# Lut99/RayTracer-3

Hardware: NVIDIA B200
Metric: Mrays/s (higher is better)
Workload: dtype f32

## Files before the change

raytracer-3_b200/csrc/rt3_core.cu:

```cuda
#include <algorithm>
#include <cmath>
#include <cstdarg>
#include <cstdio>
#include <cstdlib>
#include <cstring>
#include <atomic>
#include <chrono>
#include <limits>
#include <mutex>
#include <string>
#include <type_traits>
#include <vector>

#include <cub/device/device_radix_sort.cuh>

#include "rt3_kernels.cuh"
#include "rt3_denoise.cuh"
#include "rt3_scene.cuh"
#include "rt3_upload.cuh"

namespace {

thread_local std::string g_error;

// ... 53 lines not shown
    int sm_count = 0;
    cudaStream_t stream = nullptr;
    cudaEvent_t ev_begin = nullptr, ev_end = nullptr, ev_copy = nullptr, ev_k0 = nullptr, ev_k1 = nullptr;
    cudaStream_t last_stream = nullptr;
    bool stats_pending = false;
    bool stats_beam_accel = false;
    bool stats_beam = false;
    bool copy_timed = false;

    bool has_scene = false;
    rt3_scene_view view{};
    uint64_t scene_id = 0;
    DeviceBuffer<float4> pair_xy, filt3, face_rec, spheres, prim_color, materials;
    DeviceBuffer<float2> pair_w;
    DeviceBuffer<uint32_t> prim_material, prim_entity;

    DeviceBuffer<float4> prim_lo, prim_hi, bvh_nodes;
    float centroid_min[3] = { 0, 0, 0 }, centroid_max[3] = { 0, 0, 0 };
    bool bvh_ready = false;
    rt3_bvh_view bvh{};
    double bvh_build_ms = 0.0;

    DeviceBuffer<uint32_t> frame, aov_prim, aov_entity;
    DeviceBuffer<float> aov_t;
    DeviceBuffer<unsigned long long> aov_sums;
    DeviceBuffer<float> aov_albedo, aov_normal;
    DeviceBuffer<unsigned long long> accum, counters;
    rt3_kparams accum_kp{};
    bool accum_valid = false;
    uint32_t accum_first = 0;
// ... 104 lines not shown

template <bool RESIDENT, bool SPHERES_ONLY, bool ACCEL>
int launch_path_aovs(rt3_ctx* ctx, const rt3_camera& cam, const rt3_kparams& kp, size_t smem, uint32_t* prim, uint32_t* ent, float* t,
                     cudaStream_t stream) {
    int rc = configure(path_aov_kernel<RESIDENT, SPHERES_ONLY, ACCEL>, smem, nullptr);
    if (rc != RT3_OK) { return rc; }
    const unsigned long long per_cta = (unsigned long long) RT3_CTA_THREADS * RT3_REF_RAYS;
    const unsigned long long grid = (kp.n_items + per_cta - 1) / per_cta;
    if (grid > 0x7FFFFFFFull) { return fail(RT3_ERR_INVALID, "too many AOV samples in one call (%llu)", kp.n_items); }
    path_aov_kernel<RESIDENT, SPHERES_ONLY, ACCEL><<<(unsigned) grid, RT3_CTA_THREADS, smem, stream>>>(ctx->view, ctx->bvh, cam, kp, ctx->aov_sums.ptr, prim, ent, t,
                                                                                                     ctx->counters.ptr);
    RT3_CUDA(cudaGetLastError());
    return RT3_OK;
}

int build_bvh(rt3_ctx* ctx, cudaStream_t stream) {
    if (ctx->bvh_ready) { return RT3_OK; }
    const uint32_t count[2] = { ctx->view.n_faces, ctx->view.n_spheres }, first[2] = { 0u, ctx->view.n_faces };
    const float margin[2] = { 1.9073486328125e-06f, sqrtf(RT3_FILTER_SLACK) * 1.0001f };
    ctx->bvh.n_prims = ctx->view.n_prims;
    ctx->bvh.nodes = nullptr;
    ctx->bvh_build_ms = 0.0;
    uint32_t node_offset[2] = { 0u, count[0] > 1 ? count[0] - 1 : 0u };
    const size_t n_nodes = (size_t) node_offset[1] + (count[1] > 1 ? count[1] - 1 : 0u);
    for (int w = 0; w < 2; w++) {
        ctx->bvh.tree[w].n_prims = count[w];
        ctx->bvh.tree[w].root = count[w] == 1 ? ~(int32_t) first[w] : (int32_t) node_offset[w];
        ctx->bvh.tree[w].ray_margin = margin[w];
    }
    const uint32_t nmax = count[0] > count[1] ? count[0] : count[1];
// ... 1 lines not shown
    DeviceBuffer<unsigned long long> keys_in, keys_out;
    DeviceBuffer<uint32_t> vals_in, vals_out, arrived;
    DeviceBuffer<int> child, node_parent, leaf_parent;
    DeviceBuffer<float4> box_lo, box_hi;
    DeviceBuffer<unsigned char> temp;
    int rc;
    if ((rc = keys_in.reserve(nmax)) != RT3_OK || (rc = keys_out.reserve(nmax)) != RT3_OK || (rc = vals_in.reserve(nmax)) != RT3_OK ||
        (rc = vals_out.reserve(nmax)) != RT3_OK || (rc = arrived.reserve(nmax)) != RT3_OK || (rc = child.reserve(2 * (size_t) nmax)) != RT3_OK ||
        (rc = node_parent.reserve(nmax)) != RT3_OK || (rc = leaf_parent.reserve(nmax)) != RT3_OK || (rc = box_lo.reserve(nmax)) != RT3_OK ||
        (rc = box_hi.reserve(nmax)) != RT3_OK || (rc = ctx->bvh_nodes.reserve(4 * (n_nodes ? n_nodes : 1))) != RT3_OK) {
        return rc;
    }
    size_t temp_bytes = 0;
    RT3_CUDA(cub::DeviceRadixSort::SortPairs(nullptr, temp_bytes, keys_in.ptr, keys_out.ptr, vals_in.ptr, vals_out.ptr, (int) nmax, 0, 63, stream));
    if ((rc = temp.reserve(temp_bytes ? temp_bytes : 1)) != RT3_OK) { return rc; }
    float3 cmin = make_float3(ctx->centroid_min[0], ctx->centroid_min[1], ctx->centroid_min[2]), cscale;
    {
        const float ex[3] = { ctx->centroid_max[0] - ctx->centroid_min[0], ctx->centroid_max[1] - ctx->centroid_min[1],
                              ctx->centroid_max[2] - ctx->centroid_min[2] };
        cscale = make_float3(ex[0] > 0 ? 1.0f / ex[0] : 0.0f, ex[1] > 0 ? 1.0f / ex[1] : 0.0f, ex[2] > 0 ? 1.0f / ex[2] : 0.0f);
    }
    EventPair ev;
    if ((rc = ev.create()) != RT3_OK) { return rc; }
    RT3_CUDA(cudaEventRecord(ev.begin, stream));
    for (int w = 0; w < 2; w++) {
        const uint32_t n = count[w];
        if (n < 2) { continue; }
        const unsigned grid = (n + 255u) / 256u;
        bvh_morton_kernel<<<grid, 256, 0, stream>>>(n, first[w], ctx->prim_lo.ptr, ctx->prim_hi.ptr, cmin, cscale, keys_in.ptr, vals_in.ptr);
        RT3_CUDA(cudaGetLastError());
        size_t tb = temp_bytes;
        RT3_CUDA(cub::DeviceRadixSort::SortPairs(temp.ptr, tb, keys_in.ptr, keys_out.ptr, vals_in.ptr, vals_out.ptr, (int) n, 0, 63, stream));
        RT3_CUDA(cudaMemsetAsync(arrived.ptr, 0, (size_t) n * sizeof(uint32_t), stream));
        bvh_tree_kernel<<<grid, 256, 0, stream>>>((int) n, keys_out.ptr, child.ptr, node_parent.ptr, leaf_parent.ptr);
        RT3_CUDA(cudaGetLastError());
        bvh_refit_kernel<<<grid, 256, 0, stream>>>((int) n, vals_out.ptr, ctx->prim_lo.ptr, ctx->prim_hi.ptr, child.ptr, node_parent.ptr, leaf_parent.ptr,
// ... 3 lines not shown
    RT3_CUDA(cudaEventRecord(ev.end, stream));
    RT3_CUDA(cudaStreamSynchronize(stream));
    float ms = 0.f;
    RT3_CUDA(cudaEventElapsedTime(&ms, ev.begin, ev.end));
    ctx->bvh_build_ms = ms;
    ctx->bvh.nodes = ctx->bvh_nodes.ptr;
    ctx->bvh_ready = true;
    return RT3_OK;
}

int claim_constant_bank(rt3_ctx* ctx, cudaStream_t stream, std::unique_lock<std::mutex>& lock) {
    if (ctx->device < 0 || ctx->device >= RT3_MAX_DEVICES) { return fail(RT3_ERR_INVALID, "device %d out of range", ctx->device); }
    lock = std::unique_lock<std::mutex>(g_const_mutex[ctx->device]);
    if (g_const_owner[ctx->device] == ctx->scene_id) { return RT3_OK; }
    RT3_CUDA(cudaDeviceSynchronize());
    const size_t pairs = ctx->view.n_prims_padded / 2;
    if (pairs) {
        RT3_CUDA(cudaMemcpyToSymbolAsync(c_pair_xy, ctx->pair_xy.ptr, pairs * sizeof(float4), 0, cudaMemcpyDeviceToDevice, stream));
        RT3_CUDA(cudaMemcpyToSymbolAsync(c_pair_w, ctx->pair_w.ptr, pairs * sizeof(float2), 0, cudaMemcpyDeviceToDevice, stream));
    }
    RT3_CUDA(cudaStreamSynchronize(stream));
    g_const_owner[ctx->device] = ctx->scene_id;
    return RT3_OK;
}

struct trace_plan { bool accel, resident, spheres_only; size_t smem; };

int plan_trace(rt3_ctx* ctx, uint32_t flags, bool path_slots, cudaStream_t stream, trace_plan* plan) {
    plan->accel = (flags & RT3_FLAG_BVH) != 0;
    plan->spheres_only = ctx->view.n_faces == 0;
    if (plan->accel) {
        plan->resident = false;
        plan->smem = rt3_accel_smem_bytes(path_slots);
        return build_bvh(ctx, stream);
// ... 449 lines not shown
template <class T> int stage(DeviceBuffer<unsigned char>& buf, const T* host, size_t bytes, const T** device_view, cudaStream_t stream) {
    if (!host || bytes == 0) { *device_view = nullptr; return RT3_OK; }
    int rc = buf.reserve(bytes);
    if (rc != RT3_OK) { return rc; }
    RT3_CUDA(cudaMemcpyAsync(buf.ptr, host, bytes, cudaMemcpyHostToDevice, stream));
    *device_view = reinterpret_cast<const T*>(buf.ptr);
    return RT3_OK;
}

__global__ void build_init_kernel(rt3_build_info* info) {
    info->error_key = ~0ull; info->n_valid = 0ull; info->ray_slack = 0.f; info->r2_median = 1.0; info->r2_min = 1.0;
    for (int k = 0; k < 4; k++) { info->error_detail[k] = 0u; }
    for (int k = 0; k < 3; k++) { info->cmin_bits[k] = 0x7fffffff; info->cmax_bits[k] = (int) 0x80000000; }
}

int build_scene_on_device(rt3_ctx* ctx, const rt3_scene& d) {
    cudaStream_t stream = ctx->stream;
    ctx->has_scene = false;
    ctx->accum_valid = false;
    ctx->bvh_ready = false;
    const uint32_t nf = d.n_faces, ns = d.n_spheres, np = nf + ns;
    const uint32_t np_pad = (np + RT3_PAD_PRIMS - 1) / RT3_PAD_PRIMS * RT3_PAD_PRIMS;
    int rc;
    auto at_least_one = [](size_t n) { return n ? n : (size_t) 1; };
    if ((rc = ctx->face_rec.reserve(at_least_one(4 * (size_t) nf))) != RT3_OK ||
        (rc = ctx->spheres.reserve(at_least_one(ns))) != RT3_OK || (rc = ctx->prim_color.reserve(at_least_one(np))) != RT3_OK ||
        (rc = ctx->prim_material.reserve(at_least_one(np))) != RT3_OK || (rc = ctx->prim_entity.reserve(at_least_one(np))) != RT3_OK ||
        (rc = ctx->prim_lo.reserve(at_least_one(np))) != RT3_OK || (rc = ctx->prim_hi.reserve(at_least_one(np))) != RT3_OK ||
        (rc = ctx->filt3.reserve(at_least_one(np_pad))) != RT3_OK || (rc = ctx->pair_xy.reserve(at_least_one(np_pad / 2))) != RT3_OK ||
        (rc = ctx->pair_w.reserve(at_least_one(np_pad / 2))) != RT3_OK || (rc = ctx->materials.reserve(at_least_one((size_t) d.n_materials * 2))) != RT3_OK) {
// ... 67 lines not shown
    }
    for (int k = 0; k < 3; k++) {
        float lo = ordered_to_float(h.cmin_bits[k]), hi = ordered_to_float(h.cmax_bits[k]);
        if (!(lo <= hi)) { lo = hi = 0.0f; }
        ctx->centroid_min[k] = lo; ctx->centroid_max[k] = hi;
    }
    rt3_scene_view& v = ctx->view;
    for (int k = 0; k < 3; k++) { v.e1[k] = h.basis[0][k]; v.e2[k] = h.basis[1][k]; v.e3[k] = h.basis[2][k]; }
    v.ray_slack = h.ray_slack;
    ctx->scene_id = g_next_scene_id.fetch_add(1);
    v.n_faces = nf; v.n_spheres = ns; v.n_prims = np; v.n_prims_padded = np_pad;
    v.pair_xy = ctx->pair_xy.ptr; v.pair_w = ctx->pair_w.ptr; v.filt3 = ctx->filt3.ptr;
    v.face_rec = ctx->face_rec.ptr;
    v.spheres = ctx->spheres.ptr; v.prim_color = ctx->prim_color.ptr;
    v.prim_material = ctx->prim_material.ptr; v.prim_entity = ctx->prim_entity.ptr; v.materials = ctx->materials.ptr;
    ctx->has_scene = true;
    return RT3_OK;
}

}

extern "C" {

const char* rt3_last_error(void) { return g_error.c_str(); }

int rt3_create(rt3_ctx** out, int device) {
    if (!out) { return fail(RT3_ERR_INVALID, "out is NULL"); }
    *out = nullptr;
    int n_dev = 0;
    cudaError_t e = cudaGetDeviceCount(&n_dev);
// ... 432 lines not shown
```

raytracer-3_b200/csrc/rt3_device.cuh:

```cuda
#pragma once

#include <cuda_runtime.h>
#include <stdint.h>

#include "rt3cuda.h"
#include "rt3_rng.h"

#ifdef RT3_DEBUG_ASSERTS
#include <assert.h>
#define RT3_ASSERT(cond) assert(cond)
#else
#define RT3_ASSERT(cond) ((void) 0)
#endif

#define RT3_NO_HIT 0xFFFFFFFFu
#define RT3_TMIN 0.001f
#define RT3_ACC_SCALE 16777216.0f

#ifndef RT3_UNROLL_PAIRS
#define RT3_UNROLL_PAIRS 16
#endif
#define RT3_PRAGMA_STR(x) _Pragma(#x)
#define RT3_PRAGMA_UNROLL(n) RT3_PRAGMA_STR(unroll n)
#ifndef RT3_RAYS
#define RT3_RAYS 2
#endif
#ifndef RT3_REF_RAYS
#define RT3_REF_RAYS 2
#endif
#define RT3_WORD_PRIMS 32
#define RT3_PAD_PRIMS 8
#ifndef RT3_CHUNK_WORDS
#define RT3_CHUNK_WORDS 16
#endif
#ifndef RT3_CONST_PRIMS
#define RT3_CONST_PRIMS 768
#endif
#define RT3_TILE_PRIMS 1024
#define RT3_CTA_THREADS 128
#ifndef RT3_CTAS_PER_SM
#define RT3_CTAS_PER_SM 5
#endif
#define RT3_ITEM_CHUNK 256u
#define RT3_ITEM_CHUNK_MIN 32u

#define RT3_FILTER_SLACK 3.814697265625e-06f

struct rt3_vec3 { float x, y, z; };

__device__ __forceinline__ rt3_vec3 v3(float x, float y, float z) { rt3_vec3 r; r.x = x; r.y = y; r.z = z; return r; }
__device__ __forceinline__ rt3_vec3 operator+(rt3_vec3 a, rt3_vec3 b) { return v3(a.x + b.x, a.y + b.y, a.z + b.z); }
__device__ __forceinline__ rt3_vec3 operator-(rt3_vec3 a, rt3_vec3 b) { return v3(a.x - b.x, a.y - b.y, a.z - b.z); }
// ... 12 lines not shown
__device__ __forceinline__ uint32_t unorm8(float c) {
    float m = (c < 0.0f) ? 0.0f : c;
    m = (1.0f < m) ? 1.0f : m;
    if (m != m) { m = 0.0f; }
    return (uint32_t) roundf(m * 255.0f);
}
__device__ __forceinline__ uint32_t pack_rgb(rt3_vec3 c) {
    return (unorm8(c.x) << 24) | (unorm8(c.y) << 16) | (unorm8(c.z) << 8) | 0xFFu;
}

struct rt3_scene_view {
    uint32_t n_faces;
    uint32_t n_spheres;
    uint32_t n_prims;
    uint32_t n_prims_padded;
    const float4* pair_xy;
    const float2* pair_w;
    const float4* filt3;
    const float4* face_rec;
    const float4* spheres;
    const float4* prim_color;
    const uint32_t* prim_material;
    const uint32_t* prim_entity;
    float e1[3], e2[3], e3[3];
    float ray_slack;
    const float4* materials;
};

struct rt3_hit { float t; uint32_t prim; };

// ... 82 lines not shown

template <bool ORDERED>
__device__ __forceinline__ void exact_sphere_path_coherent(uint32_t prim, float4 sp, rt3_vec3 o, rt3_vec3 d, rt3_hit& best) {
    rt3_vec3 oc = o - v3(sp.x, sp.y, sp.z);
    float h = __fmaf_rn(oc.x, d.x, __fmaf_rn(oc.y, d.y, oc.z * d.z));
    float c = __fmaf_rn(oc.x, oc.x, __fmaf_rn(oc.y, oc.y, __fmaf_rn(oc.z, oc.z, -(sp.w * sp.w))));
    float disc = __fmaf_rn(h, h, -c);
    if (disc >= 0.0f) {
        float sq = sqrtf(disc);
        const float t1 = -h - sq, t2 = -h + sq;
        const float t = t1 >= RT3_TMIN ? t1 : t2;
        if (t >= RT3_TMIN && closer<ORDERED>(t, prim, best)) { best.prim = prim; best.t = t; }
    }
}

__constant__ float4 c_pair_xy[RT3_CONST_PRIMS / 2];
__constant__ float2 c_pair_w[RT3_CONST_PRIMS / 2];

#define RT3_MASK_BYTES_FOR(rays) ((rays) * RT3_CHUNK_WORDS * RT3_CTA_THREADS * 4)
#define RT3_MASK_BYTES RT3_MASK_BYTES_FOR(RT3_RAYS)

template <int R>
__device__ __forceinline__ void slab_pair(const float4 A, const float2 B, const float2 (&u1)[R], const float2 (&u2)[R],
                                          const float2 (&nou2)[R], uint32_t (&m)[R]) {
#pragma unroll
    for (int r = 0; r < R; r++) {
        const float2 a = __ffma2_rn(make_float2(A.x, A.y), u1[r], __ffma2_rn(make_float2(A.z, A.w), u2[r], nou2[r]));
        const float2 d = __ffma2_rn(a, a, B);
        m[r] = __funnelshift_l(__float_as_uint(d.x), m[r], 1);
        m[r] = __funnelshift_l(__float_as_uint(d.y), m[r], 1);
    }
}

template <bool CONST_BANK, int R>
__device__ __forceinline__ void sweep_chunk(const float4* __restrict__ xy, const float2* __restrict__ w, uint32_t first_pair, uint32_t n_pairs,
                                            const rt3_ray_filter (&f)[R], uint32_t* __restrict__ masks, uint32_t (&nz)[R]) {
    constexpr uint32_t WORD_PAIRS = RT3_WORD_PRIMS / 2, PAD_PAIRS = RT3_PAD_PRIMS / 2;
    float2 nou2[R], u1[R], u2[R];
#pragma unroll
    for (int r = 0; r < R; r++) {
        nou2[r] = make_float2(f[r].nou, f[r].nou); u1[r] = make_float2(f[r].u1, f[r].u1); u2[r] = make_float2(f[r].u2, f[r].u2);
        nz[r] = 0u;
    }
    uint32_t waddr = smem_u32(masks) + threadIdx.x * 4u;
    auto emit = [&](const uint32_t (&m)[R]) {
#pragma unroll
        for (int r = 0; r < R; r++) {
            asm volatile("st.shared.u32 [%0], %1;" ::"r"(waddr + (uint32_t) (r * RT3_CHUNK_WORDS * RT3_CTA_THREADS * 4)), "r"(m[r]) : "memory");
            asm("{ .reg .u32 t; add.cc.u32 t, %1, 0xFFFFFFFF; addc.u32 %0, %0, %0; }" : "+r"(nz[r]) : "r"(m[r]));
        }
        waddr += RT3_CTA_THREADS * 4u;
    };
    const uint32_t n_full = n_pairs / WORD_PAIRS;
    uint32_t base = first_pair;
    for (uint32_t wd = 0; wd < n_full; wd++, base += WORD_PAIRS) {
        uint32_t m[R];
#pragma unroll
        for (int r = 0; r < R; r++) { m[r] = 0u; }
RT3_PRAGMA_UNROLL(RT3_UNROLL_PAIRS)
        for (int j = 0; j < (int) WORD_PAIRS; j++) {
            slab_pair<R>(CONST_BANK ? c_pair_xy[base + j] : xy[base + j], CONST_BANK ? c_pair_w[base + j] : w[base + j], u1, u2, nou2, m);
        }
        emit(m);
    }
    const uint32_t left = n_pairs - n_full * WORD_PAIRS;
    if (left) {
        uint32_t m[R];
#pragma unroll
        for (int r = 0; r < R; r++) { m[r] = 0u; }
        for (uint32_t g = 0; g < left; g += PAD_PAIRS) {
#pragma unroll
            for (int j = 0; j < (int) PAD_PAIRS; j++) {
                slab_pair<R>(CONST_BANK ? c_pair_xy[base + g + j] : xy[base + g + j], CONST_BANK ? c_pair_w[base + g + j] : w[base + g + j], u1, u2, nou2, m);
            }
        }
#pragma unroll
        for (int r = 0; r < R; r++) { m[r] <<= 32u - 2u * left; }
        emit(m);
    }
}

template <bool PATH_MODE, bool SPHERES_ONLY>
__device__ __forceinline__ void drain_chunk(const rt3_scene_view& S, uint32_t first_prim, uint32_t n_words, const rt3_ray_filter& f, rt3_vec3 o,
                                            rt3_vec3 d, const uint32_t* __restrict__ masks, uint32_t nz, rt3_hit& best) {
    uint32_t m = 0u, word_prim = 0u;
    const uint32_t maddr = smem_u32(masks);
    for (;;) {
        if (m == 0u) {
            if (nz == 0u) { break; }
            const uint32_t b = 31u - (uint32_t) __clz((int) nz);
            nz ^= 1u << b;
            const uint32_t wd = n_words - 1u - b;
            RT3_ASSERT(b < n_words && n_words <= RT3_CHUNK_WORDS);
            asm volatile("ld.shared.u32 %0, [%1];" : "=r"(m) : "r"(maddr + wd * (RT3_CTA_THREADS * 4u)));
            word_prim = first_prim + wd * RT3_WORD_PRIMS;
        }
        const uint32_t k = (uint32_t) __clz((int) m);
        m ^= 0x80000000u >> k;
        const uint32_t prim = word_prim + k;
        RT3_ASSERT(prim < S.n_prims);
        if (SPHERES_ONLY || prim >= S.n_faces) {
            const float4 sp = __ldg(&S.spheres[SPHERES_ONLY ? prim : prim - S.n_faces]);
            if (PATH_MODE) { exact_sphere_path<true>(prim, sp, o, d, best); }
            else { exact_sphere_v4<true>(prim, sp, o, d, best); }
        } else {
            if (line_test(__ldg(&S.filt3[prim]), f)) { exact_face<true>(S, prim, o, d, PATH_MODE ? RT3_TMIN : 0.0f, best); }
        }
    }
}

template <bool PATH_MODE, bool CONST_BANK, bool SPHERES_ONLY, int R>
__device__ __forceinline__ void sweep_range(const rt3_scene_view& S, const float4* __restrict__ xy, const float2* __restrict__ w, uint32_t first_pair,
                                            uint32_t first_prim, uint32_t n_prims, const rt3_ray_filter (&f)[R],
                                            const rt3_vec3 (&o)[R], const rt3_vec3 (&d)[R], const bool (&live)[R],
                                            uint32_t* __restrict__ masks, rt3_hit (&best)[R]) {
    constexpr uint32_t CHUNK_PAIRS = RT3_CHUNK_WORDS * RT3_WORD_PRIMS / 2;
    const uint32_t n_pairs = n_prims / 2;
    for (uint32_t p0 = 0, w0 = 0; p0 < n_pairs; p0 += CHUNK_PAIRS, w0 += RT3_CHUNK_WORDS) {
        uint32_t nz[R];
        const uint32_t np = n_pairs - p0 < CHUNK_PAIRS ? n_pairs - p0 : CHUNK_PAIRS;
        sweep_chunk<CONST_BANK, R>(xy, w, first_pair + p0, np, f, masks, nz);
#pragma unroll
        for (int r = 0; r < R; r++) {
            if (!live[r]) { nz[r] = 0u; }
            drain_chunk<PATH_MODE, SPHERES_ONLY>(S, first_prim + w0 * RT3_WORD_PRIMS, (np + RT3_WORD_PRIMS / 2 - 1) / (RT3_WORD_PRIMS / 2), f[r], o[r], d[r],
                                                 masks + r * RT3_CHUNK_WORDS * RT3_CTA_THREADS + threadIdx.x, nz[r], best[r]);
        }
    }
}



__device__ __forceinline__ void mbar_init(uint64_t* bar, uint32_t count) {
    asm volatile("mbarrier.init.shared::cta.b64 [%0], %1;" ::"r"(smem_u32(bar)), "r"(count) : "memory");
}
__device__ __forceinline__ void mbar_expect_tx(uint64_t* bar, uint32_t bytes) {
    asm volatile("mbarrier.arrive.expect_tx.shared::cta.b64 _, [%0], %1;" ::"r"(smem_u32(bar)), "r"(bytes) : "memory");
}
__device__ __forceinline__ void mbar_wait(uint64_t* bar, uint32_t parity) {
    asm volatile(
// ... 15 lines not shown
```

raytracer-3_b200/csrc/rt3_kernels.cuh:

```cuda
#pragma once

#include "rt3_device.cuh"
#include "rt3_bvh.cuh"

struct rt3_kparams {
    uint32_t width, height;
    uint32_t spp, max_depth, seed, flags;
    uint32_t first_sample;
    uint32_t resolve_spp;
    uint32_t tile_rows, part_index, part_count;
    uint32_t owned_rows;
    unsigned long long n_pixels;
    unsigned long long n_items;
    uint32_t resident;
};

__device__ __forceinline__ uint32_t owned_row_to_global(const rt3_kparams& P, uint32_t local_row) {
    uint32_t lt = local_row / P.tile_rows, within = local_row - lt * P.tile_rows;
    return (lt * P.part_count + P.part_index) * P.tile_rows + within;
}

struct rt3_smem_view {
    uint64_t* bars;
    float4* tile_xy;
// ... 57 lines not shown
    bulk_copy_g2s(sm.tile_w + (size_t) stage * RT3_TILE_PAIRS, S.pair_w + first_pair, n * 8u, &sm.bars[stage]);
}

template <bool PATH_MODE, bool RESIDENT, bool SPHERES_ONLY, int R>
__device__ __forceinline__ void sweep_scene(const rt3_scene_view& S, const rt3_smem_view& sm, uint32_t& phase,
                                            const rt3_vec3 (&o)[R], const rt3_vec3 (&d)[R], const rt3_vec3 (&dn)[R],
                                            const bool (&live)[R], rt3_hit (&best)[R]) {
    rt3_ray_filter f[R];
#pragma unroll
    for (int r = 0; r < R; r++) {
        f[r] = make_ray_filter(S, o[r], dn[r]);
        best[r].t = __int_as_float(0x7f800000);
        best[r].prim = RT3_NO_HIT;
    }
    if (RESIDENT) {
        sweep_range<PATH_MODE, true, SPHERES_ONLY, R>(S, nullptr, nullptr, 0u, 0u, S.n_prims_padded, f, o, d, live, sm.masks, best);
        return;
    }
    const uint32_t n_tiles = (S.n_prims_padded + RT3_TILE_PRIMS - 1) / RT3_TILE_PRIMS;
    if (threadIdx.x == 0 && n_tiles > 0) { fetch_tile(S, sm, 0u, 0u); }
    for (uint32_t t = 0; t < n_tiles; t++) {
        const uint32_t stage = t & 1u;
        if (threadIdx.x == 0 && t + 1 < n_tiles) { fetch_tile(S, sm, t + 1, stage ^ 1u); }
        mbar_wait(&sm.bars[stage], (phase >> stage) & 1u);
        phase ^= 1u << stage;
        const uint32_t first = t * RT3_TILE_PRIMS;
        const uint32_t n = S.n_prims_padded - first < RT3_TILE_PRIMS ? S.n_prims_padded - first : RT3_TILE_PRIMS;
        sweep_range<PATH_MODE, false, SPHERES_ONLY, R>(S, sm.tile_xy + (size_t) stage * RT3_TILE_PAIRS, sm.tile_w + (size_t) stage * RT3_TILE_PAIRS, 0u, first, n,
                                      f, o, d, live, sm.masks, best);
        __syncthreads();
    }
// ... 21 lines not shown

#ifdef RT3_SURVIVOR_STATS
__device__ unsigned long long g_survivor_stats[4];
__device__ __forceinline__ void count_survivors(const uint32_t* __restrict__ masks, uint32_t n_words, uint32_t nz, bool live) {
    uint32_t mine = 0;
    for (uint32_t wd = 0; wd < n_words; wd++) { if ((nz >> (n_words - 1u - wd)) & 1u) { mine += (uint32_t) __popc(masks[wd * RT3_CTA_THREADS]); } }
    const uint32_t total = __reduce_add_sync(0xffffffffu, mine), most = __reduce_max_sync(0xffffffffu, mine);
    const uint32_t lanes = (uint32_t) __popc(__ballot_sync(0xffffffffu, live));
    if ((threadIdx.x & 31) == 0) {
        atomicAdd(&g_survivor_stats[0], (unsigned long long) total); atomicAdd(&g_survivor_stats[1], (unsigned long long) most);
        atomicAdd(&g_survivor_stats[2], 1ull); atomicAdd(&g_survivor_stats[3], (unsigned long long) lanes);
    }
}
#endif

template <bool SPHERES_ONLY>
__device__ __forceinline__ void drain_slots(const rt3_scene_view& S, const rt3_smem_view& sm, uint32_t first_prim, uint32_t n_pairs,
                                            const rt3_ray_filter (&f)[RT3_RAYS], const uint32_t (&nz)[RT3_RAYS]) {
    const uint32_t n_words = (n_pairs + RT3_WORD_PRIMS / 2 - 1) / (RT3_WORD_PRIMS / 2);
    static_assert(RT3_RAYS * RT3_CHUNK_WORDS <= 64, "survivor summaries are packed into 64 bits");
    unsigned long long packed = 0ull;
#pragma unroll
    for (int r = 0; r < RT3_RAYS; r++) { packed |= (unsigned long long) nz[r] << (r * RT3_CHUNK_WORDS); }
#pragma unroll 1
    for (int r = 0; r < RT3_RAYS; r++) {
        const uint32_t mine = (uint32_t) (packed >> (r * RT3_CHUNK_WORDS)) & ((1u << RT3_CHUNK_WORDS) - 1u);
        rt3_hit best;
        best.t = slot_float(sm, r, RT3_F_BEST_T); best.prim = slot_word(sm, r, RT3_F_BEST_PRIM);
        rt3_ray_filter fr = f[0];
        const rt3_vec3 o = slot_vec(sm, r, RT3_F_OX), d = slot_vec(sm, r, RT3_F_DX);
        if (!SPHERES_ONLY) { fr = make_ray_filter(S, o, d); }
#ifdef RT3_SURVIVOR_STATS
        count_survivors(sm.masks + r * RT3_CHUNK_WORDS * RT3_CTA_THREADS + threadIdx.x, n_words, mine, slot_word(sm, r, RT3_F_BOUNCE) != RT3_NO_HIT);
#endif
        drain_chunk<true, SPHERES_ONLY>(S, first_prim, n_words, fr, o, d, sm.masks + r * RT3_CHUNK_WORDS * RT3_CTA_THREADS + threadIdx.x, mine, best);
        slot_word(sm, r, RT3_F_BEST_T) = __float_as_uint(best.t); slot_word(sm, r, RT3_F_BEST_PRIM) = best.prim;
    }
}

template <bool RESIDENT, bool SPHERES_ONLY>
__device__ __forceinline__ void sweep_slots(const rt3_scene_view& S, const rt3_smem_view& sm, uint32_t& phase) {
    constexpr uint32_t CHUNK_PAIRS = RT3_CHUNK_WORDS * RT3_WORD_PRIMS / 2;
    rt3_ray_filter f[RT3_RAYS];
    slot_filters(S, sm, f);
#pragma unroll
    for (int r = 0; r < RT3_RAYS; r++) { slot_word(sm, r, RT3_F_BEST_T) = 0x7f800000u; slot_word(sm, r, RT3_F_BEST_PRIM) = RT3_NO_HIT; }
    if (RESIDENT) {
        const uint32_t n_pairs = S.n_prims_padded / 2;
        for (uint32_t p0 = 0; p0 < n_pairs; p0 += CHUNK_PAIRS) {
            uint32_t nz[RT3_RAYS];
            const uint32_t np = n_pairs - p0 < CHUNK_PAIRS ? n_pairs - p0 : CHUNK_PAIRS;
            sweep_chunk<true, RT3_RAYS>(nullptr, nullptr, p0, np, f, sm.masks, nz);
            drain_slots<SPHERES_ONLY>(S, sm, 2u * p0, np, f, nz);
        }
        return;
    }
    const uint32_t n_tiles = (S.n_prims_padded + RT3_TILE_PRIMS - 1) / RT3_TILE_PRIMS;
    if (threadIdx.x == 0 && n_tiles > 0) { fetch_tile(S, sm, 0u, 0u); }
    for (uint32_t t = 0; t < n_tiles; t++) {
        const uint32_t stage = t & 1u;
        if (threadIdx.x == 0 && t + 1 < n_tiles) { fetch_tile(S, sm, t + 1, stage ^ 1u); }
        mbar_wait(&sm.bars[stage], (phase >> stage) & 1u);
        phase ^= 1u << stage;
        const uint32_t first = t * RT3_TILE_PRIMS;
        const uint32_t n_pairs = (S.n_prims_padded - first < RT3_TILE_PRIMS ? S.n_prims_padded - first : RT3_TILE_PRIMS) / 2;
        const float4* xy = sm.tile_xy + (size_t) stage * RT3_TILE_PAIRS;
        const float2* w = sm.tile_w + (size_t) stage * RT3_TILE_PAIRS;
        for (uint32_t p0 = 0; p0 < n_pairs; p0 += CHUNK_PAIRS) {
            uint32_t nz[RT3_RAYS];
            const uint32_t np = n_pairs - p0 < CHUNK_PAIRS ? n_pairs - p0 : CHUNK_PAIRS;
            sweep_chunk<false, RT3_RAYS>(xy, w, p0, np, f, sm.masks, nz);
            drain_slots<SPHERES_ONLY>(S, sm, first + 2u * p0, np, f, nz);
        }
        __syncthreads();
    }
}

__device__ __forceinline__ uint32_t& slot_word_at(const rt3_smem_view& sm, uint32_t r, int field, uint32_t t) {
    return sm.slots[(r * RT3_SLOT_FIELDS + field) * RT3_CTA_THREADS + t];
}
__device__ __forceinline__ rt3_vec3 slot_vec_at(const rt3_smem_view& sm, uint32_t r, int field, uint32_t t) {
    return v3(__uint_as_float(slot_word_at(sm, r, field, t)), __uint_as_float(slot_word_at(sm, r, field + 1, t)), __uint_as_float(slot_word_at(sm, r, field + 2, t)));
}

#ifndef RT3_TAIL_RAYS
#define RT3_TAIL_RAYS 8
#endif
// ... 894 lines not shown
                filled += n_made;
                if (!slot_turn && !__any_sync(0xffffffffu, got)) { break; }
            }
            bool any = false;
#pragma unroll
            for (int r = 0; r < R; r++) { any = any || slot_word(sm, r, RT3_F_BOUNCE) != RT3_NO_HIT; }
            if (!__any_sync(0xffffffffu, any)) {
                if (chunk.dry) { break; }
                continue;
            }
            if constexpr (ACCEL) {
                if (BIN == 2) { traverse_slots_warp_sorted<false>(S, B, sm, bin, visits, tests); }
                else if (BIN == 3) { traverse_slots_warp_sorted<true>(S, B, sm, bin, visits, tests); }
                else { traverse_slots(S, B, sm, visits, tests); }
            } else {
                if (chunk.dry && warp_live_slots(sm) <= RT3_TAIL_RAYS) { sweep_slots_by_primitive(S, sm); }
                else { sweep_slots<RESIDENT, SPHERES_ONLY>(S, sm, phase); }
            }
        }
    } else
    for (;;) {
#pragma unroll 1
        for (int r = 0; r < R; r++) {
            rt3_path s;
            s.bounce = slot_word(sm, r, RT3_F_BOUNCE);
            if (s.bounce != RT3_NO_HIT) {
                s.o = slot_vec(sm, r, RT3_F_OX); s.d = slot_vec(sm, r, RT3_F_DX); s.thr = slot_vec(sm, r, RT3_F_TX);
                s.key = slot_word(sm, r, RT3_F_KEY); s.pix = slot_word(sm, r, RT3_F_PIX);
                rt3_hit best;
                best.t = slot_float(sm, r, RT3_F_BEST_T); best.prim = slot_word(sm, r, RT3_F_BEST_PRIM);
                rays++;
                shade_path(s, best, S, P, accum);
// ... 48 lines not shown
            }
            __syncwarp();
        }
        if (BIN == 1) {
            if (!traverse_slots_binned(S, B, sm, bin, visits, tests)) { break; }
            continue;
        }
        bool any = false;
#pragma unroll
        for (int r = 0; r < R; r++) { any = any || slot_word(sm, r, RT3_F_BOUNCE) != RT3_NO_HIT; }
        if (RESIDENT) { if (!__any_sync(0xffffffffu, any)) { break; } }
        else { if (!__syncthreads_or(any ? 1 : 0)) { break; } }
        if (BIN == 2) { traverse_slots_warp_sorted<false>(S, B, sm, bin, visits, tests); }
        else if (BIN == 3) { traverse_slots_warp_sorted<true>(S, B, sm, bin, visits, tests); }
        else if (ACCEL) { traverse_slots(S, B, sm, visits, tests); }
        else if (RESIDENT && chunk.dry && warp_live_slots(sm) <= RT3_TAIL_RAYS) { sweep_slots_by_primitive(S, sm); }
        else { sweep_slots<RESIDENT, SPHERES_ONLY>(S, sm, phase); }
    }
    for (int off = 16; off > 0; off >>= 1) { rays += __shfl_down_sync(0xffffffffu, rays, off); }
    if ((threadIdx.x & 31) == 0 && rays) { atomicAdd(&counters[1], rays); }
    if (ACCEL) { count_accel(visits, tests, counters); }
    if (BEAM) {
        unsigned long long br = beam_rays, bt = beam_tests;
        for (int off = 16; off > 0; off >>= 1) { br += __shfl_down_sync(0xffffffffu, br, off); bt += __shfl_down_sync(0xffffffffu, bt, off); }
        if ((threadIdx.x & 31) == 0 && br) { atomicAdd(&counters[ACCEL ? 5 : 2], br); atomicAdd(&counters[ACCEL ? 6 : 3], bt); }
    }
}


__device__ __forceinline__ long long to_fixed_signed(float c) {
    float s = c * RT3_ACC_SCALE;
// ... 218 lines not shown
```

raytracer-3_b200/csrc/rt3_upload.cuh:

```cuda
#pragma once

#include "rt3_device.cuh"

struct rt3_build_info {
    unsigned long long error_key;
    uint32_t error_detail[4];
    unsigned long long n_valid;
    float basis[3][3];
    float ray_slack;
    int cmin_bits[3], cmax_bits[3];
    double r2_median, r2_min;
};

#define RT3_BUILD_ERR_VERTEX 0u
#define RT3_BUILD_ERR_MATERIAL 1u
#define RT3_BUILD_ERR_KIND 2u

struct rt3_bound { double cx, cy, cz, R2; };

__device__ __forceinline__ int float_to_ordered(float f) { const int i = __float_as_int(f); return i >= 0 ? i : i ^ 0x7fffffff; }
__host__ __device__ inline float ordered_to_float(int i) {
    const int b = i >= 0 ? i : i ^ 0x7fffffff;
#if defined(__CUDA_ARCH__)
    return __int_as_float(b);
// ... 258 lines not shown
    pair_xy[j] = make_float4(a.x, b.x, a.y, b.y);
    pair_w[j] = make_float2(a.w, b.w);
#pragma unroll
    for (uint32_t k = 0; k < 2u; k++) {
        const uint32_t prim = 2u * j + k;
        if (prim >= n_prims) { continue; }
        const float4 lo = prim_lo[prim], hi = prim_hi[prim];
        if (!(lo.x <= hi.x)) { continue; }
        const float c[3] = { 0.5f * lo.x + 0.5f * hi.x, 0.5f * lo.y + 0.5f * hi.y, 0.5f * lo.z + 0.5f * hi.z };
#pragma unroll
        for (int ax = 0; ax < 3; ax++) {
            if (isfinite(c[ax])) { atomicMin(&info->cmin_bits[ax], float_to_ordered(c[ax])); atomicMax(&info->cmax_bits[ax], float_to_ordered(c[ax])); }
        }
    }
}
```

Before: 11410.

## Reorder constant bank by Morton code and cull 32-prim words via bounding spheres

Builds a constant-memory bank in which large primitives come first and the rest follow in Morton-sorted order. Each 32-primitive word gets a bounding sphere. The resident sweep first computes a per-ray reach mask against these word spheres, then skips slab testing for words no lane in the warp can reach. Drain maps bank slots back to primitive ids through a uint16 table. This is meant to cut slab work for spatially coherent scenes, at the cost of an extra per-ray word pass, an indirection load, and giving up ordered hit tie-breaking.

```diff
diff --git a/raytracer-3_b200/csrc/rt3_core.cu b/raytracer-3_b200/csrc/rt3_core.cu
--- a/raytracer-3_b200/csrc/rt3_core.cu
+++ b/raytracer-3_b200/csrc/rt3_core.cu
@@ -91,6 +91,9 @@
     DeviceBuffer<float4> pair_xy, filt3, face_rec, spheres, prim_color, materials;
     DeviceBuffer<float2> pair_w;
     DeviceBuffer<uint32_t> prim_material, prim_entity;
+    DeviceBuffer<float4> bank_xy, bank_words;
+    DeviceBuffer<float2> bank_w;
+    DeviceBuffer<uint16_t> bank_prim;
 
     DeviceBuffer<float4> prim_lo, prim_hi, bvh_nodes;
     float centroid_min[3] = { 0, 0, 0 }, centroid_max[3] = { 0, 0, 0 };
@@ -225,6 +228,13 @@
     return RT3_OK;
 }
 
+void morton_frame(const rt3_ctx* ctx, float3* cmin, float3* cscale) {
+    *cmin = make_float3(ctx->centroid_min[0], ctx->centroid_min[1], ctx->centroid_min[2]);
+    const float ex[3] = { ctx->centroid_max[0] - ctx->centroid_min[0], ctx->centroid_max[1] - ctx->centroid_min[1],
+                          ctx->centroid_max[2] - ctx->centroid_min[2] };
+    *cscale = make_float3(ex[0] > 0 ? 1.0f / ex[0] : 0.0f, ex[1] > 0 ? 1.0f / ex[1] : 0.0f, ex[2] > 0 ? 1.0f / ex[2] : 0.0f);
+}
+
 int build_bvh(rt3_ctx* ctx, cudaStream_t stream) {
     if (ctx->bvh_ready) { return RT3_OK; }
     const uint32_t count[2] = { ctx->view.n_faces, ctx->view.n_spheres }, first[2] = { 0u, ctx->view.n_faces };
@@ -256,12 +266,8 @@
     size_t temp_bytes = 0;
     RT3_CUDA(cub::DeviceRadixSort::SortPairs(nullptr, temp_bytes, keys_in.ptr, keys_out.ptr, vals_in.ptr, vals_out.ptr, (int) nmax, 0, 63, stream));
     if ((rc = temp.reserve(temp_bytes ? temp_bytes : 1)) != RT3_OK) { return rc; }
-    float3 cmin = make_float3(ctx->centroid_min[0], ctx->centroid_min[1], ctx->centroid_min[2]), cscale;
-    {
-        const float ex[3] = { ctx->centroid_max[0] - ctx->centroid_min[0], ctx->centroid_max[1] - ctx->centroid_min[1],
-                              ctx->centroid_max[2] - ctx->centroid_min[2] };
-        cscale = make_float3(ex[0] > 0 ? 1.0f / ex[0] : 0.0f, ex[1] > 0 ? 1.0f / ex[1] : 0.0f, ex[2] > 0 ? 1.0f / ex[2] : 0.0f);
-    }
+    float3 cmin, cscale;
+    morton_frame(ctx, &cmin, &cscale);
     EventPair ev;
     if ((rc = ev.create()) != RT3_OK) { return rc; }
     RT3_CUDA(cudaEventRecord(ev.begin, stream));
@@ -295,10 +301,11 @@
     lock = std::unique_lock<std::mutex>(g_const_mutex[ctx->device]);
     if (g_const_owner[ctx->device] == ctx->scene_id) { return RT3_OK; }
     RT3_CUDA(cudaDeviceSynchronize());
-    const size_t pairs = ctx->view.n_prims_padded / 2;
+    const size_t pairs = ctx->view.n_bank_recs / 2;
     if (pairs) {
-        RT3_CUDA(cudaMemcpyToSymbolAsync(c_pair_xy, ctx->pair_xy.ptr, pairs * sizeof(float4), 0, cudaMemcpyDeviceToDevice, stream));
-        RT3_CUDA(cudaMemcpyToSymbolAsync(c_pair_w, ctx->pair_w.ptr, pairs * sizeof(float2), 0, cudaMemcpyDeviceToDevice, stream));
+        RT3_CUDA(cudaMemcpyToSymbolAsync(c_pair_xy, ctx->bank_xy.ptr, pairs * sizeof(float4), 0, cudaMemcpyDeviceToDevice, stream));
+        RT3_CUDA(cudaMemcpyToSymbolAsync(c_pair_w, ctx->bank_w.ptr, pairs * sizeof(float2), 0, cudaMemcpyDeviceToDevice, stream));
+        RT3_CUDA(cudaMemcpyToSymbolAsync(c_word_sphere, ctx->bank_words.ptr, ctx->view.n_bank_words * sizeof(float4), 0, cudaMemcpyDeviceToDevice, stream));
     }
     RT3_CUDA(cudaStreamSynchronize(stream));
     g_const_owner[ctx->device] = ctx->scene_id;
@@ -778,6 +785,46 @@
     for (int k = 0; k < 3; k++) { info->cmin_bits[k] = 0x7fffffff; info->cmax_bits[k] = (int) 0x80000000; }
 }
 
+int build_bank(rt3_ctx* ctx, const rt3_bound* bounds, const rt3_build_info* info) {
+    cudaStream_t stream = ctx->stream;
+    const uint32_t n = ctx->view.n_prims;
+    DeviceBuffer<unsigned long long> keys_in, keys_out;
+    DeviceBuffer<uint32_t> vals_in, vals_out, counts;
+    DeviceBuffer<unsigned char> temp;
+    int rc;
+    if ((rc = keys_in.reserve(n)) != RT3_OK || (rc = keys_out.reserve(n)) != RT3_OK || (rc = vals_in.reserve(n)) != RT3_OK ||
+        (rc = vals_out.reserve(n)) != RT3_OK || (rc = counts.reserve(2)) != RT3_OK || (rc = ctx->bank_prim.reserve(RT3_BANK_RECS)) != RT3_OK ||
+        (rc = ctx->bank_xy.reserve(RT3_BANK_RECS / 2)) != RT3_OK || (rc = ctx->bank_w.reserve(RT3_BANK_RECS / 2)) != RT3_OK ||
+        (rc = ctx->bank_words.reserve(RT3_BANK_WORDS)) != RT3_OK) {
+        return rc;
+    }
+    size_t temp_bytes = 0;
+    RT3_CUDA(cub::DeviceRadixSort::SortPairs(nullptr, temp_bytes, keys_in.ptr, keys_out.ptr, vals_in.ptr, vals_out.ptr, (int) n, 0, 64, stream));
+    if ((rc = temp.reserve(temp_bytes ? temp_bytes : 1)) != RT3_OK) { return rc; }
+    float3 cmin, cscale;
+    morton_frame(ctx, &cmin, &cscale);
+    const unsigned grid = (n + 255u) / 256u;
+    RT3_CUDA(cudaMemsetAsync(counts.ptr, 0, 2 * sizeof(uint32_t), stream));
+    bvh_morton_kernel<<<grid, 256, 0, stream>>>(n, 0u, ctx->prim_lo.ptr, ctx->prim_hi.ptr, cmin, cscale, keys_in.ptr, vals_in.ptr);
+    RT3_CUDA(cudaGetLastError());
+    build_bank_keys_kernel<<<grid, 256, 0, stream>>>(n, bounds, info, keys_in.ptr, counts.ptr);
+    RT3_CUDA(cudaGetLastError());
+    RT3_CUDA(cub::DeviceRadixSort::SortPairs(temp.ptr, temp_bytes, keys_in.ptr, keys_out.ptr, vals_in.ptr, vals_out.ptr, (int) n, 0, 64, stream));
+    build_bank_records_kernel<<<(RT3_BANK_RECS / 2 + 127) / 128, 128, 0, stream>>>(n, vals_out.ptr, ctx->filt3.ptr, counts.ptr, ctx->bank_prim.ptr,
+                                                                                    ctx->bank_xy.ptr, ctx->bank_w.ptr);
+    RT3_CUDA(cudaGetLastError());
+    build_bank_words_kernel<<<1, 32, 0, stream>>>(counts.ptr, ctx->bank_prim.ptr, bounds, ctx->filt3.ptr, ctx->bank_words.ptr);
+    RT3_CUDA(cudaGetLastError());
+    uint32_t h[2] = { 0u, 0u };
+    RT3_CUDA(cudaMemcpyAsync(h, counts.ptr, sizeof h, cudaMemcpyDeviceToHost, stream));
+    RT3_CUDA(cudaStreamSynchronize(stream));
+    if (h[1] > RT3_BANK_RECS || h[1] < n) { return fail(RT3_ERR_INVALID, "constant-bank layout of %u records for %u primitives", h[1], n); }
+    ctx->view.n_bank_recs = h[1];
+    ctx->view.n_bank_words = (h[1] + RT3_WORD_PRIMS - 1) / RT3_WORD_PRIMS;
+    ctx->view.bank_prim = ctx->bank_prim.ptr;
+    return RT3_OK;
+}
+
 int build_scene_on_device(rt3_ctx* ctx, const rt3_scene& d) {
     cudaStream_t stream = ctx->stream;
     ctx->has_scene = false;
@@ -875,6 +922,8 @@
     v.face_rec = ctx->face_rec.ptr;
     v.spheres = ctx->spheres.ptr; v.prim_color = ctx->prim_color.ptr;
     v.prim_material = ctx->prim_material.ptr; v.prim_entity = ctx->prim_entity.ptr; v.materials = ctx->materials.ptr;
+    v.n_bank_recs = 0; v.n_bank_words = 0; v.bank_prim = nullptr;
+    if (np && np_pad <= RT3_CONST_PRIMS && (rc = build_bank(ctx, bounds.ptr, info.ptr)) != RT3_OK) { return rc; }
     ctx->has_scene = true;
     return RT3_OK;
 }
diff --git a/raytracer-3_b200/csrc/rt3_device.cuh b/raytracer-3_b200/csrc/rt3_device.cuh
--- a/raytracer-3_b200/csrc/rt3_device.cuh
+++ b/raytracer-3_b200/csrc/rt3_device.cuh
@@ -36,6 +36,9 @@
 #ifndef RT3_CONST_PRIMS
 #define RT3_CONST_PRIMS 768
 #endif
+#define RT3_BANK_RECS (RT3_CONST_PRIMS + RT3_WORD_PRIMS)
+#define RT3_BANK_WORDS (RT3_BANK_RECS / RT3_WORD_PRIMS)
+#define RT3_BANK_PAD 0xFFFFu
 #define RT3_TILE_PRIMS 1024
 #define RT3_CTA_THREADS 128
 #ifndef RT3_CTAS_PER_SM
@@ -78,6 +81,9 @@
     uint32_t n_spheres;
     uint32_t n_prims;
     uint32_t n_prims_padded;
+    uint32_t n_bank_recs;
+    uint32_t n_bank_words;
+    const uint16_t* bank_prim;
     const float4* pair_xy;
     const float2* pair_w;
     const float4* filt3;
@@ -190,8 +196,9 @@
     }
 }
 
-__constant__ float4 c_pair_xy[RT3_CONST_PRIMS / 2];
-__constant__ float2 c_pair_w[RT3_CONST_PRIMS / 2];
+__constant__ float4 c_pair_xy[RT3_BANK_RECS / 2];
+__constant__ float2 c_pair_w[RT3_BANK_RECS / 2];
+__constant__ float4 c_word_sphere[RT3_BANK_WORDS];
 
 #define RT3_MASK_BYTES_FOR(rays) ((rays) * RT3_CHUNK_WORDS * RT3_CTA_THREADS * 4)
 #define RT3_MASK_BYTES RT3_MASK_BYTES_FOR(RT3_RAYS)
@@ -208,9 +215,9 @@
     }
 }
 
-template <bool CONST_BANK, int R>
+template <bool CONST_BANK, int R, bool SKIP = false>
 __device__ __forceinline__ void sweep_chunk(const float4* __restrict__ xy, const float2* __restrict__ w, uint32_t first_pair, uint32_t n_pairs,
-                                            const rt3_ray_filter (&f)[R], uint32_t* __restrict__ masks, uint32_t (&nz)[R]) {
+                                            const rt3_ray_filter (&f)[R], uint32_t* __restrict__ masks, uint32_t (&nz)[R], uint32_t visit = ~0u) {
     constexpr uint32_t WORD_PAIRS = RT3_WORD_PRIMS / 2, PAD_PAIRS = RT3_PAD_PRIMS / 2;
     float2 nou2[R], u1[R], u2[R];
 #pragma unroll
@@ -233,9 +240,11 @@
         uint32_t m[R];
 #pragma unroll
         for (int r = 0; r < R; r++) { m[r] = 0u; }
+        if (!SKIP || __any_sync(0xffffffffu, (int) (visit << wd) < 0)) {
 RT3_PRAGMA_UNROLL(RT3_UNROLL_PAIRS)
-        for (int j = 0; j < (int) WORD_PAIRS; j++) {
-            slab_pair<R>(CONST_BANK ? c_pair_xy[base + j] : xy[base + j], CONST_BANK ? c_pair_w[base + j] : w[base + j], u1, u2, nou2, m);
+            for (int j = 0; j < (int) WORD_PAIRS; j++) {
+                slab_pair<R>(CONST_BANK ? c_pair_xy[base + j] : xy[base + j], CONST_BANK ? c_pair_w[base + j] : w[base + j], u1, u2, nou2, m);
+            }
         }
         emit(m);
     }
@@ -244,7 +253,8 @@
         uint32_t m[R];
 #pragma unroll
         for (int r = 0; r < R; r++) { m[r] = 0u; }
-        for (uint32_t g = 0; g < left; g += PAD_PAIRS) {
+        const bool any_left = !SKIP || __any_sync(0xffffffffu, (int) (visit << n_full) < 0);
+        for (uint32_t g = 0; any_left && g < left; g += PAD_PAIRS) {
 #pragma unroll
             for (int j = 0; j < (int) PAD_PAIRS; j++) {
                 slab_pair<R>(CONST_BANK ? c_pair_xy[base + g + j] : xy[base + g + j], CONST_BANK ? c_pair_w[base + g + j] : w[base + g + j], u1, u2, nou2, m);
@@ -256,9 +266,10 @@
     }
 }
 
-template <bool PATH_MODE, bool SPHERES_ONLY>
+template <bool PATH_MODE, bool SPHERES_ONLY, bool BANK>
 __device__ __forceinline__ void drain_chunk(const rt3_scene_view& S, uint32_t first_prim, uint32_t n_words, const rt3_ray_filter& f, rt3_vec3 o,
                                             rt3_vec3 d, const uint32_t* __restrict__ masks, uint32_t nz, rt3_hit& best) {
+    constexpr bool ORDERED = !BANK;
     uint32_t m = 0u, word_prim = 0u;
     const uint32_t maddr = smem_u32(masks);
     for (;;) {
@@ -273,14 +284,14 @@
         }
         const uint32_t k = (uint32_t) __clz((int) m);
         m ^= 0x80000000u >> k;
-        const uint32_t prim = word_prim + k;
+        const uint32_t prim = BANK ? (uint32_t) __ldg(&S.bank_prim[word_prim + k]) : word_prim + k;
         RT3_ASSERT(prim < S.n_prims);
         if (SPHERES_ONLY || prim >= S.n_faces) {
             const float4 sp = __ldg(&S.spheres[SPHERES_ONLY ? prim : prim - S.n_faces]);
-            if (PATH_MODE) { exact_sphere_path<true>(prim, sp, o, d, best); }
-            else { exact_sphere_v4<true>(prim, sp, o, d, best); }
+            if (PATH_MODE) { exact_sphere_path<ORDERED>(prim, sp, o, d, best); }
+            else { exact_sphere_v4<ORDERED>(prim, sp, o, d, best); }
         } else {
-            if (line_test(__ldg(&S.filt3[prim]), f)) { exact_face<true>(S, prim, o, d, PATH_MODE ? RT3_TMIN : 0.0f, best); }
+            if (line_test(__ldg(&S.filt3[prim]), f)) { exact_face<ORDERED>(S, prim, o, d, PATH_MODE ? RT3_TMIN : 0.0f, best); }
         }
     }
 }
@@ -299,7 +310,7 @@
 #pragma unroll
         for (int r = 0; r < R; r++) {
             if (!live[r]) { nz[r] = 0u; }
-            drain_chunk<PATH_MODE, SPHERES_ONLY>(S, first_prim + w0 * RT3_WORD_PRIMS, (np + RT3_WORD_PRIMS / 2 - 1) / (RT3_WORD_PRIMS / 2), f[r], o[r], d[r],
+            drain_chunk<PATH_MODE, SPHERES_ONLY, CONST_BANK>(S, first_prim + w0 * RT3_WORD_PRIMS, (np + RT3_WORD_PRIMS / 2 - 1) / (RT3_WORD_PRIMS / 2), f[r], o[r], d[r],
                                                  masks + r * RT3_CHUNK_WORDS * RT3_CTA_THREADS + threadIdx.x, nz[r], best[r]);
         }
     }
diff --git a/raytracer-3_b200/csrc/rt3_kernels.cuh b/raytracer-3_b200/csrc/rt3_kernels.cuh
--- a/raytracer-3_b200/csrc/rt3_kernels.cuh
+++ b/raytracer-3_b200/csrc/rt3_kernels.cuh
@@ -95,7 +95,7 @@
         best[r].prim = RT3_NO_HIT;
     }
     if (RESIDENT) {
-        sweep_range<PATH_MODE, true, SPHERES_ONLY, R>(S, nullptr, nullptr, 0u, 0u, S.n_prims_padded, f, o, d, live, sm.masks, best);
+        sweep_range<PATH_MODE, true, SPHERES_ONLY, R>(S, nullptr, nullptr, 0u, 0u, S.n_bank_recs, f, o, d, live, sm.masks, best);
         return;
     }
     const uint32_t n_tiles = (S.n_prims_padded + RT3_TILE_PRIMS - 1) / RT3_TILE_PRIMS;
@@ -147,7 +147,7 @@
 }
 #endif
 
-template <bool SPHERES_ONLY>
+template <bool SPHERES_ONLY, bool BANK>
 __device__ __forceinline__ void drain_slots(const rt3_scene_view& S, const rt3_smem_view& sm, uint32_t first_prim, uint32_t n_pairs,
                                             const rt3_ray_filter (&f)[RT3_RAYS], const uint32_t (&nz)[RT3_RAYS]) {
     const uint32_t n_words = (n_pairs + RT3_WORD_PRIMS / 2 - 1) / (RT3_WORD_PRIMS / 2);
@@ -166,28 +166,71 @@
 #ifdef RT3_SURVIVOR_STATS
         count_survivors(sm.masks + r * RT3_CHUNK_WORDS * RT3_CTA_THREADS + threadIdx.x, n_words, mine, slot_word(sm, r, RT3_F_BOUNCE) != RT3_NO_HIT);
 #endif
-        drain_chunk<true, SPHERES_ONLY>(S, first_prim, n_words, fr, o, d, sm.masks + r * RT3_CHUNK_WORDS * RT3_CTA_THREADS + threadIdx.x, mine, best);
+        drain_chunk<true, SPHERES_ONLY, BANK>(S, first_prim, n_words, fr, o, d, sm.masks + r * RT3_CHUNK_WORDS * RT3_CTA_THREADS + threadIdx.x, mine, best);
         slot_word(sm, r, RT3_F_BEST_T) = __float_as_uint(best.t); slot_word(sm, r, RT3_F_BEST_PRIM) = best.prim;
     }
 }
 
+__device__ __forceinline__ void word_reach(const rt3_scene_view& S, const rt3_smem_view& sm, uint32_t (&reach)[RT3_RAYS]) {
+    float ox[RT3_RAYS], oy[RT3_RAYS], oz[RT3_RAYS], dx[RT3_RAYS], dy[RT3_RAYS], dz[RT3_RAYS], omega[RT3_RAYS];
+#pragma unroll
+    for (int r = 0; r < RT3_RAYS; r++) {
+        ox[r] = slot_float(sm, r, RT3_F_OX); oy[r] = slot_float(sm, r, RT3_F_OY); oz[r] = slot_float(sm, r, RT3_F_OZ);
+        dx[r] = slot_float(sm, r, RT3_F_DX); dy[r] = slot_float(sm, r, RT3_F_DY); dz[r] = slot_float(sm, r, RT3_F_DZ);
+        const float dd = __fmaf_rn(dx[r], dx[r], __fmaf_rn(dy[r], dy[r], dz[r] * dz[r]));
+        omega[r] = __fmaf_rn(S.ray_slack, __fmaf_rn(ox[r], ox[r], __fmaf_rn(oy[r], oy[r], oz[r] * oz[r])), 1.0f);
+        if (!(fabsf(dd - 1.0f) <= 9.5367431640625e-07f)) { omega[r] = __int_as_float(0x7fc00000); }
+        reach[r] = 0u;
+    }
+#pragma unroll 1
+    for (uint32_t k = 0; k < S.n_bank_words; k++) {
+        const float4 w = c_word_sphere[k];
+#pragma unroll
+        for (int r = 0; r < RT3_RAYS; r++) {
+            const float cx = w.x - ox[r], cy = w.y - oy[r], cz = w.z - oz[r];
+            const float tc = __fmaf_rn(cx, dx[r], __fmaf_rn(cy, dy[r], cz * dz[r]));
+            const float L = __fmaf_rn(cx, cx, __fmaf_rn(cy, cy, cz * cz));
+            const float lim = __fmaf_rn(L, 1.52587890625e-05f, w.w * omega[r]);
+            const bool drop = __fmaf_rn(-tc, tc, L) > lim || (tc < 0.0f && L > lim);
+            reach[r] = 2u * reach[r] + (drop ? 0u : 1u);
+        }
+    }
+#pragma unroll
+    for (int r = 0; r < RT3_RAYS; r++) {
+        reach[r] = S.n_bank_words ? reach[r] << (32u - S.n_bank_words) : 0u;
+        if (slot_word(sm, r, RT3_F_BOUNCE) == RT3_NO_HIT) { reach[r] = 0u; }
+    }
+}
+
 template <bool RESIDENT, bool SPHERES_ONLY>
-__device__ __forceinline__ void sweep_slots(const rt3_scene_view& S, const rt3_smem_view& sm, uint32_t& phase) {
+__device__ __forceinline__ void sweep_slots(const rt3_scene_view& S, const rt3_smem_view& sm, uint32_t& phase, bool done = false) {
     constexpr uint32_t CHUNK_PAIRS = RT3_CHUNK_WORDS * RT3_WORD_PRIMS / 2;
     rt3_ray_filter f[RT3_RAYS];
     slot_filters(S, sm, f);
-#pragma unroll
-    for (int r = 0; r < RT3_RAYS; r++) { slot_word(sm, r, RT3_F_BEST_T) = 0x7f800000u; slot_word(sm, r, RT3_F_BEST_PRIM) = RT3_NO_HIT; }
     if (RESIDENT) {
-        const uint32_t n_pairs = S.n_prims_padded / 2;
-        for (uint32_t p0 = 0; p0 < n_pairs; p0 += CHUNK_PAIRS) {
+        uint32_t reach[RT3_RAYS], visit = 0u;
+        word_reach(S, sm, reach);
+#pragma unroll
+        for (int r = 0; r < RT3_RAYS; r++) {
+            if (done) { reach[r] = 0u; }
+            else { slot_word(sm, r, RT3_F_BEST_T) = 0x7f800000u; slot_word(sm, r, RT3_F_BEST_PRIM) = RT3_NO_HIT; }
+            visit |= reach[r];
+        }
+
+        const uint32_t n_pairs = S.n_bank_recs / 2;
+        for (uint32_t p0 = 0, w0 = 0; p0 < n_pairs; p0 += CHUNK_PAIRS, w0 += RT3_CHUNK_WORDS) {
             uint32_t nz[RT3_RAYS];
             const uint32_t np = n_pairs - p0 < CHUNK_PAIRS ? n_pairs - p0 : CHUNK_PAIRS;
-            sweep_chunk<true, RT3_RAYS>(nullptr, nullptr, p0, np, f, sm.masks, nz);
-            drain_slots<SPHERES_ONLY>(S, sm, 2u * p0, np, f, nz);
+            const uint32_t n_words = (np + RT3_WORD_PRIMS / 2 - 1) / (RT3_WORD_PRIMS / 2);
+            sweep_chunk<true, RT3_RAYS, true>(nullptr, nullptr, p0, np, f, sm.masks, nz, visit << w0);
+#pragma unroll
+            for (int r = 0; r < RT3_RAYS; r++) { nz[r] &= (reach[r] << w0) >> (32u - n_words); }
+            drain_slots<SPHERES_ONLY, true>(S, sm, 2u * p0, np, f, nz);
         }
         return;
     }
+#pragma unroll
+    for (int r = 0; r < RT3_RAYS; r++) { slot_word(sm, r, RT3_F_BEST_T) = 0x7f800000u; slot_word(sm, r, RT3_F_BEST_PRIM) = RT3_NO_HIT; }
     const uint32_t n_tiles = (S.n_prims_padded + RT3_TILE_PRIMS - 1) / RT3_TILE_PRIMS;
     if (threadIdx.x == 0 && n_tiles > 0) { fetch_tile(S, sm, 0u, 0u); }
     for (uint32_t t = 0; t < n_tiles; t++) {
@@ -203,7 +246,7 @@
             uint32_t nz[RT3_RAYS];
             const uint32_t np = n_pairs - p0 < CHUNK_PAIRS ? n_pairs - p0 : CHUNK_PAIRS;
             sweep_chunk<false, RT3_RAYS>(xy, w, p0, np, f, sm.masks, nz);
-            drain_slots<SPHERES_ONLY>(S, sm, first + 2u * p0, np, f, nz);
+            drain_slots<SPHERES_ONLY, false>(S, sm, first + 2u * p0, np, f, nz);
         }
         __syncthreads();
     }
@@ -1128,8 +1171,9 @@
                 else if (BIN == 3) { traverse_slots_warp_sorted<true>(S, B, sm, bin, visits, tests); }
                 else { traverse_slots(S, B, sm, visits, tests); }
             } else {
-                if (chunk.dry && warp_live_slots(sm) <= RT3_TAIL_RAYS) { sweep_slots_by_primitive(S, sm); }
-                else { sweep_slots<RESIDENT, SPHERES_ONLY>(S, sm, phase); }
+                const bool tail = chunk.dry && warp_live_slots(sm) <= RT3_TAIL_RAYS;
+                if (tail) { sweep_slots_by_primitive(S, sm); }
+                sweep_slots<RESIDENT, SPHERES_ONLY>(S, sm, phase, tail);
             }
         }
     } else
@@ -1208,7 +1252,11 @@
         if (BIN == 2) { traverse_slots_warp_sorted<false>(S, B, sm, bin, visits, tests); }
         else if (BIN == 3) { traverse_slots_warp_sorted<true>(S, B, sm, bin, visits, tests); }
         else if (ACCEL) { traverse_slots(S, B, sm, visits, tests); }
-        else if (RESIDENT && chunk.dry && warp_live_slots(sm) <= RT3_TAIL_RAYS) { sweep_slots_by_primitive(S, sm); }
+        else if (RESIDENT) {
+            const bool tail = chunk.dry && warp_live_slots(sm) <= RT3_TAIL_RAYS;
+            if (tail) { sweep_slots_by_primitive(S, sm); }
+            sweep_slots<RESIDENT, SPHERES_ONLY>(S, sm, phase, tail);
+        }
         else { sweep_slots<RESIDENT, SPHERES_ONLY>(S, sm, phase); }
     }
     for (int off = 16; off > 0; off >>= 1) { rays += __shfl_down_sync(0xffffffffu, rays, off); }
diff --git a/raytracer-3_b200/csrc/rt3_upload.cuh b/raytracer-3_b200/csrc/rt3_upload.cuh
--- a/raytracer-3_b200/csrc/rt3_upload.cuh
+++ b/raytracer-3_b200/csrc/rt3_upload.cuh
@@ -296,3 +296,67 @@
         }
     }
 }
+
+#define RT3_BANK_LARGE_R2 16.0
+
+__global__ void build_bank_keys_kernel(uint32_t n, const rt3_bound* __restrict__ bounds, const rt3_build_info* __restrict__ info,
+                                       unsigned long long* __restrict__ keys, uint32_t* __restrict__ n_large) {
+    const uint32_t i = blockIdx.x * blockDim.x + threadIdx.x;
+    if (i >= n) { return; }
+    const bool large = bounds[i].R2 > RT3_BANK_LARGE_R2 * info->r2_median;
+    keys[i] = large ? 0ull : keys[i] + 1ull;
+    if (large) { atomicAdd(n_large, 1u); }
+}
+
+__global__ void build_bank_records_kernel(uint32_t n, const uint32_t* __restrict__ sorted, const float4* __restrict__ filt3, uint32_t* __restrict__ n_large,
+                                          uint16_t* __restrict__ bank_prim, float4* __restrict__ bank_xy, float2* __restrict__ bank_w) {
+    const uint32_t j = blockIdx.x * blockDim.x + threadIdx.x;
+    const uint32_t nl = n_large[0], first_small = (nl + RT3_WORD_PRIMS - 1) / RT3_WORD_PRIMS * RT3_WORD_PRIMS;
+    const uint32_t n_recs = (first_small + (n - nl) + RT3_PAD_PRIMS - 1) / RT3_PAD_PRIMS * RT3_PAD_PRIMS;
+    if (j == 0) { n_large[1] = n_recs; }
+    if (2u * j >= n_recs) { return; }
+    const float4 never = make_float4(0.f, 0.f, 0.f, __int_as_float(0x7f800000));
+    float4 rec[2];
+#pragma unroll
+    for (uint32_t h = 0; h < 2u; h++) {
+        const uint32_t k = 2u * j + h;
+        const uint32_t at = k < nl ? k : k < first_small ? n : nl + (k - first_small);
+        const uint32_t prim = at < n ? sorted[at] : RT3_BANK_PAD;
+        bank_prim[k] = (uint16_t) prim;
+        rec[h] = prim != RT3_BANK_PAD ? filt3[prim] : never;
+    }
+    bank_xy[j] = make_float4(rec[0].x, rec[1].x, rec[0].y, rec[1].y);
+    bank_w[j] = make_float2(rec[0].w, rec[1].w);
+}
+
+__global__ void build_bank_words_kernel(const uint32_t* __restrict__ n_large, const uint16_t* __restrict__ bank_prim, const rt3_bound* __restrict__ bounds,
+                                        const float4* __restrict__ filt3, float4* __restrict__ words) {
+    const uint32_t wd = blockIdx.x * blockDim.x + threadIdx.x;
+    if (wd >= RT3_BANK_WORDS || wd * RT3_WORD_PRIMS >= n_large[1]) { return; }
+    const uint32_t k0 = wd * RT3_WORD_PRIMS, k1 = min(k0 + RT3_WORD_PRIMS, n_large[1]);
+    double lo[3] = { 1e300, 1e300, 1e300 }, hi[3] = { -1e300, -1e300, -1e300 };
+    auto member = [&](uint32_t k, double c[3], double* R) {
+        const uint32_t prim = bank_prim[k];
+        if (prim == RT3_BANK_PAD) { return false; }
+        const float w = filt3[prim].w;
+        if (!(w <= 0.f)) { return false; }
+        const rt3_bound b = bounds[prim];
+        c[0] = b.cx; c[1] = b.cy; c[2] = b.cz; *R = sqrt(-(double) w);
+        return true;
+    };
+    for (uint32_t k = k0; k < k1; k++) {
+        double c[3], R;
+        if (!member(k, c, &R)) { continue; }
+        for (int a = 0; a < 3; a++) { lo[a] = fmin(lo[a], c[a]); hi[a] = fmax(hi[a], c[a]); }
+    }
+    if (!(lo[0] <= hi[0])) { words[wd] = make_float4(0.f, 0.f, 0.f, -__int_as_float(0x7f800000)); return; }
+    const float C[3] = { (float) (0.5 * (lo[0] + hi[0])), (float) (0.5 * (lo[1] + hi[1])), (float) (0.5 * (lo[2] + hi[2])) };
+    const double Cd[3] = { C[0], C[1], C[2] };
+    double W = 0.0;
+    for (uint32_t k = k0; k < k1; k++) {
+        double c[3], R;
+        if (!member(k, c, &R)) { continue; }
+        W = fmax(W, dist3(c, Cd) + R);
+    }
+    words[wd] = make_float4(C[0], C[1], C[2], round_up_f(W * W * (1.0 + 1e-12)));
+}
```

After: 10430 (median of 6 runs). -8.6%, worse.
